# nicolapiccinelli/libmpc

Hardware: AMD Instinct MI355X
Metric: MPC solves/sec (whole node) + p50 solve latency, quadrotor LMPC N=20 batch=4096 (higher is better)
Workload: dtype f64; 1 GPU; quadrotor_ex.cpp LMPC nx=12 nu=4 ny=12 ph=ch=20, batch 4096 per GPU, SplitMix64 x0/u0/yref (SURVEY 8d), maximum_iteration=250; parallelism=single GPU, rccl_ranks=0, streams=1

## Files before the change

include/mpcx.h:

```cpp
#ifndef MPCX_H
#define MPCX_H

#include <stdint.h>

#ifdef __cplusplus
extern "C" {
#endif

#define MPCX_OK              0
#define MPCX_E_INVALID      -1
#define MPCX_E_UNSUPPORTED  -2
#define MPCX_E_DEVICE       -3
#define MPCX_E_NUMERIC      -4
#define MPCX_E_STATE        -5

#define MPCX_STATUS_SUCCESS        0
#define MPCX_STATUS_MAX_ITERATION  1
#define MPCX_STATUS_INFEASIBLE     2
#define MPCX_STATUS_ERROR          3
#define MPCX_STATUS_UNKNOWN        4

#define MPCX_SOLVER_SOLVED               1
#define MPCX_SOLVER_SOLVED_INACCURATE    2
#define MPCX_SOLVER_MAX_ITER_REACHED    -2
// ... 211 lines not shown

#define MPCX_COMM_ID_BYTES 128
typedef struct mpcx_comm *mpcx_comm_t;
int mpcx_comm_get_unique_id(void *id_out );
int mpcx_comm_create(int device, int rank, int world, const void *id, mpcx_comm_t *out);
int mpcx_comm_destroy(mpcx_comm_t c);
int mpcx_comm_rank(mpcx_comm_t c);
int mpcx_comm_world(mpcx_comm_t c);
int mpcx_allgather_u(mpcx_comm_t c, const double *u_local, int rows_per_rank, int nu, double *u_all, void *stream);

typedef struct mpcx_lmpc_hetero *mpcx_lmpc_hetero_t;
int mpcx_lmpc_hetero_create(const mpcx_lmpc_t *controllers, int count, int device, mpcx_lmpc_hetero_t *out);
int mpcx_lmpc_hetero_create_ex(const mpcx_lmpc_t *controllers, int count, int device, int condense_on_host, mpcx_lmpc_hetero_t *out);
int mpcx_lmpc_hetero_destroy(mpcx_lmpc_hetero_t f);
int mpcx_lmpc_hetero_get_info(mpcx_lmpc_hetero_t f, int *count, int *active_words, int *m_ref, double *bytes_per_model);
int mpcx_lmpc_hetero_solve_batch(mpcx_lmpc_hetero_t f, const mpcx_lmpc_batch *b, const int32_t *model_index, void *stream);
int mpcx_lmpc_hetero_time_solve_batch(mpcx_lmpc_hetero_t f, const mpcx_lmpc_batch *b, const int32_t *model_index, void *stream,
                                      int repeats, float *ms_mean);

int mpcx_lmpc_set_total_batch(mpcx_lmpc_t h, int total);

int mpcx_lmpc_debug_time_kernels(mpcx_lmpc_t h, const mpcx_lmpc_batch *b, void *stream, int repeats, float *ms3);
int mpcx_lmpc_debug_get(mpcx_lmpc_t h, const char *name, double *out, int cap);
int mpcx_lmpc_debug_setup_counts(mpcx_lmpc_t h, int *full, int *refs);
int mpcx_lmpc_debug_use_fused(mpcx_lmpc_t h, int mode);
int mpcx_lmpc_debug_force_generic(mpcx_lmpc_t h, int on);
int mpcx_lmpc_debug_set_rounds(mpcx_lmpc_t h, int rounds0, int check_every);
int mpcx_lmpc_debug_set_cycle_buffer(mpcx_lmpc_t h, void *dev_ptr);
int mpcx_lmpc_loop_debug_replay(mpcx_lmpc_loop_t l, void *stream);
int mpcx_lmpc_loop_debug_tick(mpcx_lmpc_loop_t l, int *tick);
int mpcx_nlmpc_debug_set_tolerances(mpcx_nlmpc_t h, double tol_step, double tol_con);
int mpcx_nlmpc_debug_last_form(void);
int mpcx_nlmpc_last_form(mpcx_nlmpc_t h);
int mpcx_nlmpc_debug_get_ws(mpcx_nlmpc_t h, int instance, double *out, int cap, int *layout, int nlayout);
int mpcx_nlmpc_debug_generated_source(const mpcx_nlmpc_source *src, char *out, int cap);
int mpcx_nlmpc_debug_compile_source(const mpcx_nlmpc_source *src);
int mpcx_lmpc_hetero_debug_get(mpcx_lmpc_hetero_t f, int k, const char *name, double *out, int cap);

const char *mpcx_version(void);

#ifdef __cplusplus
}
#endif
#endif
```

libmpc_amd/_capi.py:

```python
from __future__ import annotations

import ctypes as C
import os

_HERE = os.path.dirname(os.path.abspath(__file__))
LIB_PATH = os.environ.get("MPCX_LIBRARY", os.path.join(_HERE, "libmpcx.so"))

OK = 0
E_INVALID, E_UNSUPPORTED, E_DEVICE, E_NUMERIC, E_STATE = -1, -2, -3, -4, -5
STATUS_SUCCESS, STATUS_MAX_ITERATION, STATUS_INFEASIBLE, STATUS_ERROR, STATUS_UNKNOWN = range(5)
REF_SHARED, REF_PER_INSTANCE, REF_PER_STEP = 0, 1, 2
REF_PREVIEW = 3


class Dims(C.Structure):
    _fields_ = [(n, C.c_int) for n in ("nx", "nu", "ndu", "ny", "ph", "ch")]


class LParams(C.Structure):
    _fields_ = [("maximum_iteration", C.c_int), ("time_limit", C.c_double), ("enable_warm_start", C.c_int),
                ("alpha", C.c_double), ("rho", C.c_double), ("eps_rel", C.c_double), ("eps_abs", C.c_double),
                ("eps_prim_inf", C.c_double), ("eps_dual_inf", C.c_double),
                ("verbose", C.c_int), ("adaptive_rho", C.c_int), ("polish", C.c_int)]

# ... 36 lines not shown


EXPORTS = [
    "mpcx_lmpc_create", "mpcx_lmpc_destroy", "mpcx_lparams_default", "mpcx_last_error",
    "mpcx_lmpc_set_state_space_model", "mpcx_lmpc_set_disturbances",
    "mpcx_lmpc_set_objective_weights", "mpcx_lmpc_set_objective_weights_slice",
    "mpcx_lmpc_set_state_bounds", "mpcx_lmpc_set_state_bounds_slice",
    "mpcx_lmpc_set_input_bounds", "mpcx_lmpc_set_input_bounds_slice",
    "mpcx_lmpc_set_output_bounds", "mpcx_lmpc_set_output_bounds_slice",
    "mpcx_lmpc_set_scalar_constraint_slice", "mpcx_lmpc_set_scalar_constraint_index",
    "mpcx_lmpc_set_references", "mpcx_lmpc_set_references_slice",
    "mpcx_lmpc_set_exogenous_inputs", "mpcx_lmpc_set_exogenous_inputs_slice",
    "mpcx_lmpc_set_optimizer_parameters", "mpcx_lmpc_set_strict_infeasibility", "mpcx_lmpc_setup", "mpcx_lmpc_solve_batch",
    "mpcx_lmpc_time_solve_batch", "mpcx_lmpc_solve_host", "mpcx_lmpc_get_info", "mpcx_version",
    "mpcx_lmpc_graph_create", "mpcx_lmpc_graph_launch", "mpcx_lmpc_graph_destroy",
    "mpcx_lmpc_loop_create", "mpcx_lmpc_loop_run", "mpcx_lmpc_loop_destroy", "mpcx_lmpc_loop_desc_size",
    "mpcx_nlmpc_create", "mpcx_nlmpc_destroy", "mpcx_nlmpc_get_dims", "mpcx_nlmpc_evaluate_batch",
    "mpcx_nlparams_default", "mpcx_nlmpc_set_optimizer_parameters", "mpcx_nlmpc_solve_batch", "mpcx_nlmpc_time_solve_batch", "mpcx_discretize_batch",
    "mpcx_nlmpc_set_state_bounds_slice", "mpcx_nlmpc_set_input_bounds_slice", "mpcx_nlmpc_solve_host",
    "mpcx_nlmpc_create_custom", "mpcx_nlmpc_create_from_source", "mpcx_nlmpc_set_input_scale", "mpcx_nlmpc_set_state_scale",
    "mpcx_comm_get_unique_id", "mpcx_comm_create", "mpcx_comm_destroy", "mpcx_comm_rank", "mpcx_comm_world", "mpcx_allgather_u",
    "mpcx_lmpc_hetero_create", "mpcx_lmpc_hetero_destroy", "mpcx_lmpc_hetero_get_info", "mpcx_lmpc_hetero_solve_batch",
    "mpcx_lmpc_hetero_time_solve_batch", "mpcx_lmpc_hetero_create_ex", "mpcx_lmpc_hetero_debug_get",
    "mpcx_lmpc_set_total_batch", "mpcx_lmpc_debug_time_kernels", "mpcx_lmpc_debug_get", "mpcx_lmpc_debug_setup_counts", "mpcx_lmpc_debug_use_fused",
    "mpcx_lmpc_debug_force_generic", "mpcx_lmpc_debug_set_rounds", "mpcx_lmpc_debug_set_cycle_buffer",
    "mpcx_lmpc_loop_debug_replay", "mpcx_lmpc_loop_debug_tick",
    "mpcx_nlmpc_debug_set_tolerances", "mpcx_nlmpc_debug_last_form", "mpcx_nlmpc_last_form", "mpcx_nlmpc_debug_get_ws", "mpcx_nlmpc_debug_generated_source", "mpcx_nlmpc_debug_compile_source",
]


class NLParams(C.Structure):
    _fields_ = [("maximum_iteration", C.c_int), ("time_limit", C.c_double), ("enable_warm_start", C.c_int),
                ("relative_ftol", C.c_double), ("relative_xtol", C.c_double), ("absolute_ftol", C.c_double),
                ("absolute_xtol", C.c_double), ("hard_constraints", C.c_int)]


class NlmpcBatch(C.Structure):
    _fields_ = [("batch", C.c_int), ("x0", C.c_void_p), ("u0", C.c_void_p), ("z_warm", C.c_void_p), ("cmd", C.c_void_p),
                ("cost", C.c_void_p), ("status", C.c_void_p), ("solver_status", C.c_void_p), ("is_feasible", C.c_void_p),
                ("iterations", C.c_void_p), ("z", C.c_void_p), ("seq_state", C.c_void_p), ("seq_input", C.c_void_p),
                ("seq_output", C.c_void_p), ("warm_curvature", C.c_int), ("multipliers", C.c_void_p), ("params", C.c_void_p)]


class NlmpcDims(C.Structure):
    _fields_ = [(n, C.c_int) for n in ("nx", "nu", "ph", "ch", "nz", "neq", "nineq", "jeq_w", "neq_user", "ny", "nbnd", "n_params")]


# ... 65 lines not shown
```

libmpc_amd/csrc/lmpc_device.hpp:

```cpp
#pragma once

#include <atomic>
#include <cstdint>
#include <initializer_list>

namespace mpcx {

constexpr int kMaxActive = 28;
constexpr int kSld = kMaxActive + 1;
__host__ __device__ inline int ws_capacity(int nz) { return nz > kMaxActive ? nz : kMaxActive; }

struct LmpcDev {
    int nx, nu, ndu, ny, ph, ch, nf, nz, mg;
    int ldz, ldg, ldy;
    int m_ref, neq_ref, active_words;
    int has_dist, n_fixed;
    int max_iter, polish, check_every, polish_rounds0, polish_rounds;
    int cost_direct;
    int cond_status;
    int strict_infeasible;
    double alpha, sigma, eps_abs, eps_rel, eps_prim_inf;
    int adaptive_rho; double rho_user;
    int stage_len, arena_len, lds_per_wave;
    int fast_slice;
    int wsld;
    const double *A, *B, *C, *Bd, *Dd;
    const double *Wy, *Wu, *Wdu;
    const double *yref_s, *uref_s, *duref_s, *dmeas_s;
    const double *lo0x, *hi0x, *lo0u, *hi0u, *lo0y, *hi0y, *sX, *sU;
    double s0lo, s0hi;
    const double *H, *Kinv, *Gr, *Gc, *Y;
    const double *lw, *uw, *rho_b;
    const double *lg0, *ug0, *rho_g;
    const int *g_kind, *g_step, *g_comp, *g_refrow;
    const int *f_kind, *f_step, *f_comp; const double *f_lo, *f_hi;
    const int *boxrow_ptr, *boxrow_ref; const double *boxrow_lo, *boxrow_hi;
    const int *blk;
    int kin, nxp, nup, nyp, ione, nz16, mg16, ns, ns16, kq16, rowsA, ldy16;
    const double *MA0, *MA1, *Ym, *slo, *shi;
    const double *MA0p, *MA1p, *Ymp;
    const double *Hp;
    int rowsF, nsp, fused_ok, group_ok;
    const double *MF0, *MF1;
};

struct LmpcBatchDev {
    int batch;
    const double *x0, *u0;
    const double *yref; long yref_bs, yref_ks;
    const double *uref; long uref_bs, uref_ks;
    const double *duref; long duref_bs, duref_ks;
    const double *dmeas; long dmeas_bs, dmeas_ks;
    double *cmd, *cost;
    int32_t *status, *solver_status, *is_feasible, *iterations;
    uint32_t *active_lower, *active_upper;
    double *seq_state, *seq_output, *seq_input;
    int32_t *polish_rounds, *active_count;
    const uint32_t *warm_lower, *warm_upper;
    int warm_shift;
    int fq_cap;
    int fused;
    int *fq;
    int *pcounter;
    int n_models;
    const int32_t *model_index;
    long long *dbg_cycles;
// ... 59 lines not shown
```

libmpc_amd/csrc/lmpc_fast.hip:

```cpp
#include "lmpc_kernel_common.hpp"
#include <cstddef>
#include <cstdlib>
#include <utility>

namespace mpcx {

namespace {

#ifndef MPCX_FAST_PF_MAXCAP
#define MPCX_FAST_PF_MAXCAP 12
#endif
#ifndef MPCX_FAST_RB
#define MPCX_FAST_RB 4
#endif
#ifndef MPCX_FAST_PF
#define MPCX_FAST_PF 4
#endif
#ifndef MPCX_FAST_PF_ALL
#define MPCX_FAST_PF_ALL 6
#endif
#ifndef MPCX_FAST_NBUF
#define MPCX_FAST_NBUF 3
#endif
#ifndef MPCX_FAST_RB_DEEP
// ... 937 lines not shown
        const gdp src = gl(Bt.fused == 2 ? M.MF1 : M.MF0);
        for (int k = 2 * (int)threadIdx.x; k < nmf; k += 2 * (int)blockDim.x) {
            const d2 v = ld2(src + k);
            *reinterpret_cast<double2 *>(smem + k) = make_double2(v.x, v.y);
        }
    }
    double *lwuw = smem + nmf;
    fast_load_box<CPZ>(M, lwuw);
    double *rec = lwuw + 2 * 128 * CPZ + (size_t)wave * M.fast_slice;
    const int nwaves = gridDim.x * kPersistWaves, shard = blockIdx.x & 7;
    int b = blockIdx.x * kPersistWaves + wave;
    while (b < Bt.batch) {
        solve_fast<CPZ, CPG, 1>(M, Bt, b, lane, rec, lwuw, glw(wsbase) + (size_t)b * M.wsld, smem);
        int n = 0;
        if (lane == 0) n = atomicAdd(counter + shard, 1);
        n = __builtin_amdgcn_readfirstlane(n);
        b = nwaves + shard + 8 * n;
    }
}

template <size_t BYTES>
__device__ __forceinline__ void kernarg_touch()
{
    static_assert(BYTES <= 16 * 64 && BYTES > 15 * 64, "kernarg_touch covers sixteen lines, the sixteenth must exist");
    const auto ka = __builtin_amdgcn_kernarg_segment_ptr();
    int t0, t1, t2, t3, t4, t5, t6, t7, t8, t9, t10, t11, t12, t13, t14, t15;
    asm volatile("s_load_dword %0, %16, 0x0\n\ts_load_dword %1, %16, 0x40\n\ts_load_dword %2, %16, 0x80\n\ts_load_dword %3, %16, 0xc0\n\t"
                 "s_load_dword %4, %16, 0x100\n\ts_load_dword %5, %16, 0x140\n\ts_load_dword %6, %16, 0x180\n\ts_load_dword %7, %16, 0x1c0\n\t"
                 "s_load_dword %8, %16, 0x200\n\ts_load_dword %9, %16, 0x240\n\ts_load_dword %10, %16, 0x280\n\ts_load_dword %11, %16, 0x2c0\n\t"
                 "s_load_dword %12, %16, 0x300\n\ts_load_dword %13, %16, 0x340\n\ts_load_dword %14, %16, 0x380\n\ts_load_dword %15, %16, 0x3c0\n\t"
                 "s_waitcnt lgkmcnt(0)"
                 : "=&s"(t0), "=&s"(t1), "=&s"(t2), "=&s"(t3), "=&s"(t4), "=&s"(t5), "=&s"(t6), "=&s"(t7), "=&s"(t8), "=&s"(t9), "=&s"(t10), "=&s"(t11),
                   "=&s"(t12), "=&s"(t13), "=&s"(t14), "=&s"(t15)
                 : "s"(ka)
                 : "memory");
}
#ifndef MPCX_GROUP_BALANCE
#define MPCX_GROUP_BALANCE 1
#endif

template <int CPZ> constexpr int kGroupWavesOf = CPZ == 1 ? 16 : 8;
constexpr int kGroupG2 = 5;
constexpr int kGroupG1 = 2;
template <int CPZ, int CPG>
__global__ __launch_bounds__(kGroupWavesOf<CPZ> * 64) void lmpc_solve_group(const LmpcDev Mv, const LmpcBatchDev Btv, double *wsbasev, const int variantv)
{
    constexpr int kGroupWaves = kGroupWavesOf<CPZ>;
    extern __shared__ __attribute__((aligned(16))) double smem[];
#if defined(MPCX_GROUP_CUT) && MPCX_GROUP_CUT == 0
    { return; }
#endif
    kernarg_touch<sizeof(LmpcDev) + sizeof(LmpcBatchDev) + sizeof(double *) + sizeof(int)>();
    const group_args_p ka = (group_args_p)__builtin_amdgcn_kernarg_segment_ptr();
    const LmpcDev &M = (const LmpcDev &)ka->M;
    const LmpcBatchDev &Bt = (const LmpcBatchDev &)ka->Bt;
    double *const wsbase = ka->wsbase;
    const int variant = ka->variant;
    const int lane = threadIdx.x & 63, wave = threadIdx.x >> 6;
    const int j = lane & 15, kq = lane >> 4;
    const int nx = M.nx, nu = M.nu, ny = M.ny;
    const int kin4 = M.kin >> 2, nz4 = M.nz16 >> 2;
    const int ldz = M.ldz, ldg = M.ldg, ldy = M.ldy;
    constexpr int ZP = 128 * CPZ, GPD = 128 * CPG;
    double *lwuw = smem;
    double *slices = lwuw + 2 * ZP;
    double *Bv = slices + (size_t)kGroupWaves * M.fast_slice;
    double *Bf = Bv + (size_t)kin4 * 64;
    double *c0s = Bf + (size_t)nz4 * 64;
    unsigned *bad = reinterpret_cast<unsigned *>(c0s + kGroupWaves * 16);
    const int outld = 8 + ((nu + 1) & ~1);
    double *outs = c0s + kGroupWaves * 16 + 16;
    double *mine = slices + (size_t)wave * M.fast_slice;
    const gdp MAp = gl(variant ? M.MA1p : M.MA0p), Ymp = GP(Ymp);
    const int ntile1 = M.rowsA >> 4, tg = M.nz16 >> 4, ts = tg + (M.mg16 >> 4), tq = ts + (M.ns16 >> 4);
    const int ntile2 = M.ldy16 >> 4;
    const int G1 = (kin4 + 3) >> 2, G2 = (nz4 + 3) >> 2;
    auto ld4 = [](gdp p) -> v4d { return *reinterpret_cast<const v4d MPCX_GAS *>(p); };
    const bool jlive = j < kGroupWaves;
    double *sj = slices + (size_t)(jlive ? j : 0) * M.fast_slice;
    double *t0j = sj, *gt0j = sj + ZP, *lgj = gt0j + GPD, *ugj = lgj + GPD, *fj = ugj + GPD;

    const int b0 = blockIdx.x * kGroupWaves;
    const int bj = b0 + (jlive ? j : kGroupWaves - 1);
    const int bc = bj < Bt.batch ? bj : Bt.batch - 1;
    auto gstamp = [&](int k) { if (Bt.dbg_cycles && lane == 0 && b0 + wave < Bt.batch) Bt.dbg_cycles[(size_t)(b0 + wave) * 8 + k] = (long long)__builtin_readcyclecounter(); };
    gstamp(4);

    auto vin_at = [&](int kb) -> double {
        const int k = 4 * kb + kq;
        gdp src = gl(Bt.x0);
        bool ld = false;
        if (k < M.nxp) { ld = k < nx; src = gl(Bt.x0) + ((size_t)bc * nx + k); }
        else if (k < M.nxp + M.nup) { const int c = k - M.nxp; ld = c < nu; src = gl(Bt.u0) + ((size_t)bc * nu + c); }
        else if (k < M.ione) { const int c = k - M.nxp - M.nup; ld = variant && c < ny; src = gl(Bt.yref) + ((size_t)bc * Bt.yref_bs + c); }
        double v = k == M.ione ? 1.0 : 0.0;
        if (ld) v = *src;
        return v;
    };
    const double vin0 = wave < kin4 ? vin_at(wave) : 0.0;
    const int ebx = 2 * (int)threadIdx.x;
    const bool boxok = ebx < ldz;
    d2 bxl = {0.0, 0.0}, bxu = {0.0, 0.0};
    if (ebx < ZP) { bxl = ld2(GP(lw) + (boxok ? ebx : 0)); bxu = ld2(GP(uw) + (boxok ? ebx : 0)); }
    const int t1 = wave < ntile1 ? wave : ntile1 - 1;
    v4d a1[kGroupG1];
#pragma unroll
    for (int g = 0; g < kGroupG1; ++g) a1[g] = ld4(MAp + (((size_t)t1 * G1 + (g < G1 ? g : 0)) * 64 + lane) * 4);
    double eblo[4], ebhi[4];
    {
        const bool ing = t1 >= tg && t1 < ts, ins = t1 >= ts && t1 < tq;
        const gdp plo = ing ? GP(lg0) + 16 * (t1 - tg) : GP(slo) + 16 * (ins ? t1 - ts : 0);
        const gdp phi = ing ? GP(ug0) + 16 * (t1 - tg) : GP(shi) + 16 * (ins ? t1 - ts : 0);
        const int lim = ing ? ldg - 16 * (t1 - tg) : (ins ? M.ns - 16 * (t1 - ts) : 0);
#pragma unroll
        for (int r = 0; r < 4; ++r) {
            const int row = 4 * r + kq;
            eblo[r] = 0.0; ebhi[r] = 0.0;
            if (row < lim) { eblo[r] = plo[row]; ebhi[r] = phi[row]; }
        }
    }
    const int t2 = wave < ntile2 ? wave : ntile2 - 1;
    v4d a2[kGroupG2];
#pragma unroll
    for (int g = 0; g < kGroupG2; ++g) a2[g] = ld4(Ymp + (((size_t)t2 * G2 + (g < G2 ? g : 0)) * 64 + lane) * 4);
    d2 eql[CPG], equ[CPG];
#pragma unroll
    for (int c = 0; c < CPG; ++c) {
        const int r = 128 * c + 2 * lane;
        eql[c] = d2{0.0, 0.0}; equ[c] = d2{1.0, 1.0};
        if (wave == kGroupWaves - 1) { eql[c] = ld2(GP(lg0) + (r < ldg ? r : 0)); equ[c] = ld2(GP(ug0) + (r < ldg ? r : 0)); }
    }

    fast_init_pads<CPZ, CPG>(mine, ldz, ldg, lane);
    if (wave < kin4) Bv[wave * 64 + lane] = vin0;
    for (int kb = wave + kGroupWaves; kb < kin4; kb += kGroupWaves) Bv[kb * 64 + lane] = vin_at(kb);
    if (ebx < ZP) {
        const double INF = __builtin_huge_val();
        *reinterpret_cast<double2 *>(lwuw + ebx) = boxok ? make_double2(bxl.x, bxl.y) : make_double2(-INF, -INF);
        *reinterpret_cast<double2 *>(lwuw + ZP + ebx) = boxok ? make_double2(bxu.x, bxu.y) : make_double2(INF, INF);
    }
    if (threadIdx.x < 16) bad[threadIdx.x] = 0u;
    __syncthreads();
    gstamp(7);
#if defined(MPCX_GROUP_CUT) && MPCX_GROUP_CUT == 1
// ... 25 lines not shown
                    if (jlive && row < ldz) fj[row] = acc[r];
                }
            } else if (t < ts) {
#pragma unroll
                for (int r = 0; r < 4; ++r) {
                    const int row = 16 * (t - tg) + 4 * r + kq;
                    if (jlive && row < ldg) {
                        const double l0 = PRE ? eblo[r] : GP(lg0)[row], u0 = PRE ? ebhi[r] : GP(ug0)[row];
                        lgj[row] = l0 - acc[r]; ugj[row] = u0 - acc[r];
                    }
                }
            } else if (t < tq) {
#pragma unroll
                for (int r = 0; r < 4; ++r) {
                    const int row = 16 * (t - ts) + 4 * r + kq;
                    if (row < M.ns) badl |= violates(acc[r], PRE ? eblo[r] : GP(slo)[row], PRE ? ebhi[r] : GP(shi)[row], M.eps_abs, M.eps_rel);
                }
            } else {
#pragma unroll
                for (int r = 0; r < 4; ++r) {
                    const int kb2 = 4 * (t - tq) + r;
                    if (kb2 < kin4) c0p = fma(0.5 * Bv[kb2 * 64 + lane], acc[r], c0p);
                }
            }
        };
        int *eqb = reinterpret_cast<int *>(outs + kGroupWaves * outld);
        if (wave < ntile1) tile1.template operator()<true>(wave);
        for (int t = wave + kGroupWaves; t < ntile1; t += kGroupWaves) tile1.template operator()<false>(t);
        if (badl && jlive) atomicOr(&bad[j], 1u);
        c0p += __shfl_xor(c0p, 16, 64);
        c0p += __shfl_xor(c0p, 32, 64);
        if (kq == 0) c0s[wave * 16 + j] = c0p;
        __syncthreads();
        gstamp(5);
#if defined(MPCX_GROUP_CUT) && MPCX_GROUP_CUT == 2
        { return; }
#endif

        auto tile2 = [&]<bool PRE>(const int t) {
            v4d acc = {0.0, 0.0, 0.0, 0.0};
            for (int g0 = 0; g0 < G2; g0 += kGroupG2) {
                v4d a[kGroupG2];
#pragma unroll
                for (int g = 0; g < kGroupG2; ++g) a[g] = (PRE && g0 == 0) ? a2[g] : ld4(Ymp + (((size_t)t * G2 + (g0 + g < G2 ? g0 + g : g0)) * 64 + lane) * 4);
#pragma unroll
                for (int g = 0; g < kGroupG2; ++g)
#pragma unroll
                    for (int e = 0; e < 4; ++e) {
                        const int kb = 4 * (g0 + g) + e;
                        if (kb < nz4) acc = __builtin_amdgcn_mfma_f64_16x16x4f64(a[g][e], Bf[kb * 64 + lane], acc, 0, 0, 0);
                    }
            }
#pragma unroll
            for (int r = 0; r < 4; ++r) {
                const int row = 16 * t + 4 * r + kq;
                if (!jlive) continue;
                if (row < ldz) t0j[row] = acc[r];
                else if (row < ldy) gt0j[row - ldz] = acc[r];
            }
        };
        if (wave < ntile2) tile2.template operator()<true>(wave);
        for (int t = wave + kGroupWaves; t < ntile2; t += kGroupWaves) tile2.template operator()<false>(t);
        if (wave == kGroupWaves - 1) {
            int bits = 0;
#pragma unroll
            for (int c = 0; c < CPG; ++c) {
                const bool ok = 128 * c + 2 * lane < ldg;
                bits |= ((ok && eql[c].x == equ[c].x) ? 1 : 0) << (2 * c) | ((ok && eql[c].y == equ[c].y) ? 1 : 0) << (2 * c + 1);
            }
            eqb[lane] = bits;
        }
        if (threadIdx.x < kGroupWaves) {
            double *tl = slices + (size_t)threadIdx.x * M.fast_slice + 2 * ZP + 3 * GPD;
            double c0 = 0.0;
            for (int w = 0; w < kGroupWaves; ++w) c0 += c0s[w * 16 + threadIdx.x];
            tl[0] = c0;
            tl[1] = bad[threadIdx.x] ? 1.0 : 0.0;
        }
        __syncthreads();
        const int eqbits = eqb[lane];
        int inst = wave;
#if MPCX_GROUP_BALANCE
        if (b0 + kGroupWaves <= Bt.batch) {
            const double *t0m = mine, *gt0m = mine + ZP, *lgm = gt0m + GPD, *ugm = lgm + GPD;
            auto over = [](double v, double lo, double hi) { return fmax(fmax(lo - v, v - hi), 0.0); };
            double sv = 0.0;
#pragma unroll
            for (int c = 0; c < CPZ; ++c) {
                const int e = 128 * c + 2 * lane;
                const double2 l = *reinterpret_cast<const double2 *>(lwuw + e), u = *reinterpret_cast<const double2 *>(lwuw + ZP + e), t = *reinterpret_cast<const double2 *>(t0m + e);
                sv += over(t.x, l.x, u.x) + over(t.y, l.y, u.y);
            }
#pragma unroll
            for (int c = 0; c < CPG; ++c) {
                const int r = 128 * c + 2 * lane;
                const double2 l = *reinterpret_cast<const double2 *>(lgm + r), u = *reinterpret_cast<const double2 *>(ugm + r), t = *reinterpret_cast<const double2 *>(gt0m + r);
                sv += over(t.x, l.x, u.x) + over(t.y, l.y, u.y);
            }
            sv = wave_sum(sv);
            double *keys = reinterpret_cast<double *>(bad);
            if (lane == 0) keys[wave] = sv;
            __syncthreads();
            const int me = lane & (kGroupWaves - 1), part = lane >> 4;
            const double ki = keys[me];
            int rank = 0;
#pragma unroll
            for (int q = 0; q < kGroupWaves / 4; ++q) {
                const int jj = (kGroupWaves / 4) * part + q;
                const double kj = keys[jj];
                rank += (kj > ki || (kj == ki && jj < me)) ? 1 : 0;
            }
            rank += __shfl_xor(rank, 16, 64);
            rank += __shfl_xor(rank, 32, 64);
            const int q = rank >> 2, sd = (q & 1) ? 3 - (rank & 3) : (rank & 3);
            inst = (int)__builtin_ctzll(__ballot(lane < kGroupWaves && 4 * q + sd == wave));
        }
#endif
        double *const slice_i = slices + (size_t)inst * M.fast_slice;
        const int b = b0 + inst;
        gstamp(6);
#if defined(MPCX_GROUP_CUT) && MPCX_GROUP_CUT == 3
        { return; }
#endif
        if (b < Bt.batch) solve_fast<CPZ, CPG, 2>(M, Bt, b, lane, slice_i, lwuw, glw(wsbase) + (size_t)b * M.wsld, nullptr, outs + inst * outld, eqbits);
        __syncthreads();
        {
            const int t = threadIdx.x;
            if (t < kGroupWaves && b0 + t < Bt.batch) {
                const double *o = outs + t * outld;
                const int bb = b0 + t;
                if (o[7] == 2.0) {
                    if (Bt.cost) glw(Bt.cost)[bb] = o[0];
                    if (Bt.status) glw(Bt.status)[bb] = (int)o[1];
                    if (Bt.solver_status) glw(Bt.solver_status)[bb] = (int)o[2];
                    if (Bt.is_feasible) glw(Bt.is_feasible)[bb] = (int)o[3];
                    if (Bt.iterations) glw(Bt.iterations)[bb] = 0;
                    if (Bt.polish_rounds) glw(Bt.polish_rounds)[bb] = (int)o[5];
                    if (Bt.active_count) glw(Bt.active_count)[bb] = (int)o[6];
                }
            }
            for (int e = t; e < kGroupWaves * nu; e += blockDim.x) {
                const int ti = e / nu, jj = e - ti * nu;
// ... 60 lines not shown
    else if (b.n_models > 0) hipLaunchKernelGGL(k2h, dim3(blocks), dim3(kWavesPerBlock * 64), ldsf, stream, m_dev, b, ws);
    else hipLaunchKernelGGL(k2, dim3(blocks), dim3(kWavesPerBlock * 64), ldsf, stream, m_dev, b, ws);
    return hipGetLastError() == hipSuccess ? 0 : -3;
}

}

int lmpc_fast_slice(const LmpcDev &m)
{
    const int cp = lmpc_kernel_variant(m.ldz, m.ldg);
    if (cp < 1) return 0;
    const int fixed = cp == 1 ? fast_slice_fixed<1, 1>() : (cp == 2 ? fast_slice_fixed<2, 2>() : fast_slice_fixed<4, 4>());
    const int scratch = m.kin > 2 * m.nx ? m.kin : 2 * m.nx;
    int n = (fixed + scratch + 1) / 2 * 2;
    while (n % 16 != 2) n += 2;
    return n;
}

size_t lmpc_group_lds_bytes(const LmpcDev &m)
{
    const int cp = lmpc_kernel_variant(m.ldz, m.ldg);
    if (cp != 1 && cp != 2) return 0;
    const int nw = cp == 1 ? 16 : 8;
    return ((size_t)2 * 128 * cp + (size_t)nw * m.fast_slice + (size_t)(m.kin / 4 + m.nz16 / 4) * 64 + (size_t)nw * 16 + 16 + (size_t)nw * (8 + ((m.nu + 1) & ~1)) + 32) * sizeof(double);
}

int lmpc_launch_fast(const LmpcDev &m, const LmpcDev *m_dev, const LmpcBatchDev &b, double *ws, void *stream, LmpcForm form)
{
    hipStream_t s = reinterpret_cast<hipStream_t>(stream);
    switch (lmpc_kernel_variant(m.ldz, m.ldg)) {
    case 1: return launch_fast_variant<1, 1>(m, m_dev, b, ws, s, form);
#ifndef MPCX_FAST_ONLY_CP1
    case 2: return launch_fast_variant<2, 2>(m, m_dev, b, ws, s, form);
    case 4: return launch_fast_variant<4, 4>(m, m_dev, b, ws, s, form);
#endif
    default: return -2;
    }
}

}
```

libmpc_amd/csrc/mpcx_capi.cpp:

```cpp
#include <hip/hip_runtime.h>

#include <cstdio>
#include <cstring>
#include <memory>
#include <atomic>
#include <chrono>
#include <string>
#include <thread>
#include <type_traits>
#include <vector>

#include "../../include/mpcx.h"
#include "lmpc_device.hpp"
#include "lmpc_model.hpp"

namespace {

thread_local std::string g_err;

int fail(int code, const std::string &msg)
{
    g_err = msg;
    return code;
}
// ... 118 lines not shown
    D.nz16 = o.nz16; D.mg16 = o.mg16; D.ns = o.ns; D.ns16 = o.ns16; D.kq16 = o.kq16; D.rowsA = o.rowsA; D.ldy16 = o.ldy16;
    D.fast_slice = mpcx::lmpc_fast_slice(D);
    D.MA0 = U.up(o.MA[0], rc); D.MA1 = U.up(o.MA[1], rc); D.Ym = U.up(o.Ym, rc);
    {
        std::vector<double> pk;
        auto packed = [&](const std::vector<double> &v, int rows, int K) -> const std::vector<double> & {
            pk.clear();
            if (!v.empty()) { pk.resize(mpcx::lmpc_packed_len(rows, K)); mpcx::lmpc_pack_mfma_tiles(v.data(), rows, K, pk.data()); }
            return pk;
        };
        D.MA0p = U.up(packed(o.MA[0], o.rowsA, o.kin), rc); D.MA1p = U.up(packed(o.MA[1], o.rowsA, o.kin), rc); D.Ymp = U.up(packed(o.Ym, o.ldy16, o.nz16), rc);
        std::vector<double> hpad;
        if (D.cost_direct && !o.MA[0].empty() && !o.H.empty()) {
            hpad.assign((size_t)o.nz16 * o.nz16, 0.0);
            for (int c = 0; c < o.nz; ++c)
                for (int r = 0; r < o.nz; ++r) hpad[(size_t)c * o.nz16 + r] = o.H[(size_t)c * o.ldz + r];
        }
        D.Hp = hpad.empty() ? nullptr : U.up(packed(hpad, o.nz16, o.nz16), rc);
    }
    D.MF0 = U.up(o.MF[0], rc); D.MF1 = U.up(o.MF[1], rc); D.rowsF = o.rowsF; D.nsp = o.nsp;
    D.fused_ok = (h->use_fused != 0 && mpcx::lmpc_kernel_variant(o.ldz, o.ldg) == 1 && o.rowsF <= 384 && !D.cost_direct) ? 1 : 0;
    const size_t ldsg = mpcx::lmpc_group_lds_bytes(D);
    const int cpv = mpcx::lmpc_kernel_variant(o.ldz, o.ldg);
    D.group_ok = (h->use_fused != 0 && ldsg > 0 && ldsg <= mpcx::lmpc_lds_limit() && ((cpv == 1 && !D.cost_direct) || (cpv == 2 && h->use_fused == 2))) ? 1 : 0;
    D.slo = U.up(o.slo, rc); D.shi = U.up(o.shi, rc);
}

struct SlabUploader {
    static constexpr size_t kDevRegion = (size_t)1 << 44;
    std::vector<char> host;
    size_t dev_bytes = 0;
    bool big_on_device = false;
    template <typename T>
    const T *up(const std::vector<T> &v, int &)
    {
        const size_t at = (host.size() + 15) / 16 * 16;
        host.resize(at + (v.size() ? v.size() : 1) * sizeof(T), 0);
        if (v.size()) std::memcpy(host.data() + at, v.data(), v.size() * sizeof(T));
        return reinterpret_cast<const T *>(at + 1);
    }
    const double *reserve_big(size_t n)
    {
        const size_t at = (dev_bytes + 15) / 16 * 16;
        dev_bytes = at + (n ? n : 1) * sizeof(double);
        return reinterpret_cast<const double *>(kDevRegion + at + 1);
    }
    template <typename T>
// ... 1068 lines not shown

int mpcx_lmpc_debug_force_generic(mpcx_lmpc_t h, int on)
{
    CHECK_H(h);
    h->force_generic = on != 0;
    return MPCX_OK;
}

int mpcx_lmpc_debug_set_rounds(mpcx_lmpc_t h, int rounds0, int check_every)
{
    CHECK_H(h);
    h->dbg_rounds0 = rounds0; h->dbg_check_every = check_every;
    h->dirty = true;
    return MPCX_OK;
}

int mpcx_lmpc_debug_set_cycle_buffer(mpcx_lmpc_t h, void *dev_ptr)
{
    CHECK_H(h);
    h->dbg_cycles = static_cast<long long *>(dev_ptr);
    return MPCX_OK;
}

int mpcx_lmpc_debug_get(mpcx_lmpc_t h, const char *name, double *out, int cap)
{
    CHECK_H(h);
    int rc = mpcx_lmpc_setup(h);
    if (rc != MPCX_OK) return rc;
    const auto &o = h->cond;
    const std::vector<double> *v = nullptr;
    std::vector<double> tmp;
    std::string n(name ? name : "");
    if (n == "H") v = &o.H; else if (n == "Kinv") v = &o.Kinv; else if (n == "Gr") v = &o.Gr;
    else if (n == "Gc") v = &o.Gc; else if (n == "Y") v = &o.Y; else if (n == "lw") v = &o.lw;
    else if (n == "uw") v = &o.uw; else if (n == "rho_b") v = &o.rho_b; else if (n == "lg0") v = &o.lg0;
    else if (n == "ug0") v = &o.ug0; else if (n == "rho_g") v = &o.rho_g;
    else if (n == "dims") {
        tmp = {(double)o.nz, (double)o.mg, (double)o.ldz, (double)o.ldg, (double)o.ldy, (double)o.nf,
               (double)o.n_ref, (double)o.m_ref, (double)o.neq_ref, (double)o.fixed_rows.size(),
               (double)h->dev.lds_per_wave, (double)(o.h_regularised ? 1 : 0)};
        v = &tmp;
    } else if (n == "MA0") v = &o.MA[0]; else if (n == "MA1") v = &o.MA[1]; else if (n == "Ym") v = &o.Ym;
    else if (n == "MA0p" || n == "MA1p" || n == "Ymp") {
        const std::vector<double> &src = n == "Ymp" ? o.Ym : o.MA[n == "MA1p" ? 1 : 0];
        const int rows = n == "Ymp" ? o.ldy16 : o.rowsA, K = n == "Ymp" ? o.nz16 : o.kin;
        if (!src.empty()) { tmp.resize(mpcx::lmpc_packed_len(rows, K)); mpcx::lmpc_pack_mfma_tiles(src.data(), rows, K, tmp.data()); }
        v = &tmp;
    } else if (n == "flags") {
        tmp = {(double)h->dev.cost_direct, (double)h->dev.group_ok, (double)h->dev.fused_ok};
        v = &tmp;
    } else if (n == "dims_maps") {
        tmp = {(double)o.kin, (double)o.nxp, (double)o.nup, (double)o.nyp, (double)o.ione, (double)o.nz16, (double)o.mg16,
               (double)o.ns, (double)o.ns16, (double)o.kq16, (double)o.rowsA, (double)o.ldy16};
        v = &tmp;
    } else if (n == "g_refrow") { tmp.assign(o.g_refrow.begin(), o.g_refrow.end()); v = &tmp; }
    else if (n == "g_step") { tmp.assign(o.g_step.begin(), o.g_step.end()); v = &tmp; }
    else if (n == "g_kind") { tmp.assign(o.g_kind.begin(), o.g_kind.end()); v = &tmp; }
    else if (n == "g_comp") { tmp.assign(o.g_comp.begin(), o.g_comp.end()); v = &tmp; }
    else if (n == "fallback") {
        tmp.assign(3, 0.0);
        if (out && !h->host_only) {
            if (hipSetDevice(h->device) != hipSuccess || !fallback_state(h->scratch, tmp.data())) return fail(MPCX_E_DEVICE, "hipMemcpy failed");
        }
        v = &tmp;
    }
    else return fail(MPCX_E_INVALID, "unknown array name");
    if (!out) return (int)v->size();
    if (cap < (int)v->size()) return fail(MPCX_E_INVALID, "buffer too small");
    std::memcpy(out, v->data(), sizeof(double) * v->size());
    return (int)v->size();
}

}
// ... 1 lines not shown
```

Baseline: 126.4 million solves/s.

## Phase group-kernel tile work with host-built load-balanced schedule across waves

Splits the first matrix-tile phase so that only the tiles feeding the next stage run before the barrier. The remaining phase-1 tiles are interleaved with phase-2 tiles according to a greedy, SIMD-balanced schedule computed on the host and passed through kernel arguments. Balance keys are computed inside the tile-2 epilogue instead of a separate pass, and the cross-row reductions use permlane swaps instead of shuffles. The cost is a larger kernarg block (one more cache line to touch), extra LDS, per-tile reductions of the constant term, and a fallback path when the schedule does not fit.

```diff
diff --git a/include/mpcx.h b/include/mpcx.h
--- a/include/mpcx.h
+++ b/include/mpcx.h
@@ -257,6 +257,7 @@
 
 int mpcx_lmpc_debug_time_kernels(mpcx_lmpc_t h, const mpcx_lmpc_batch *b, void *stream, int repeats, float *ms3);
 int mpcx_lmpc_debug_get(mpcx_lmpc_t h, const char *name, double *out, int cap);
+int mpcx_lmpc_debug_group_schedule(int ts, int ntile1, int ntile2, int kin4, int nz4, int waves, unsigned char *out64);
 int mpcx_lmpc_debug_setup_counts(mpcx_lmpc_t h, int *full, int *refs);
 int mpcx_lmpc_debug_use_fused(mpcx_lmpc_t h, int mode);
 int mpcx_lmpc_debug_force_generic(mpcx_lmpc_t h, int on);
diff --git a/libmpc_amd/_capi.py b/libmpc_amd/_capi.py
--- a/libmpc_amd/_capi.py
+++ b/libmpc_amd/_capi.py
@@ -82,7 +82,7 @@
     "mpcx_comm_get_unique_id", "mpcx_comm_create", "mpcx_comm_destroy", "mpcx_comm_rank", "mpcx_comm_world", "mpcx_allgather_u",
     "mpcx_lmpc_hetero_create", "mpcx_lmpc_hetero_destroy", "mpcx_lmpc_hetero_get_info", "mpcx_lmpc_hetero_solve_batch",
     "mpcx_lmpc_hetero_time_solve_batch", "mpcx_lmpc_hetero_create_ex", "mpcx_lmpc_hetero_debug_get",
-    "mpcx_lmpc_set_total_batch", "mpcx_lmpc_debug_time_kernels", "mpcx_lmpc_debug_get", "mpcx_lmpc_debug_setup_counts", "mpcx_lmpc_debug_use_fused",
+    "mpcx_lmpc_set_total_batch", "mpcx_lmpc_debug_time_kernels", "mpcx_lmpc_debug_get", "mpcx_lmpc_debug_group_schedule", "mpcx_lmpc_debug_setup_counts", "mpcx_lmpc_debug_use_fused",
     "mpcx_lmpc_debug_force_generic", "mpcx_lmpc_debug_set_rounds", "mpcx_lmpc_debug_set_cycle_buffer",
     "mpcx_lmpc_loop_debug_replay", "mpcx_lmpc_loop_debug_tick",
     "mpcx_nlmpc_debug_set_tolerances", "mpcx_nlmpc_debug_last_form", "mpcx_nlmpc_last_form", "mpcx_nlmpc_debug_get_ws", "mpcx_nlmpc_debug_generated_source", "mpcx_nlmpc_debug_compile_source",
diff --git a/libmpc_amd/csrc/lmpc_device.hpp b/libmpc_amd/csrc/lmpc_device.hpp
--- a/libmpc_amd/csrc/lmpc_device.hpp
+++ b/libmpc_amd/csrc/lmpc_device.hpp
@@ -3,6 +3,8 @@
 #include <atomic>
 #include <cstdint>
 #include <initializer_list>
+
+#include "lmpc_group_schedule.hpp"
 
 namespace mpcx {
 
@@ -42,6 +44,7 @@
     const double *Hp;
     int rowsF, nsp, fused_ok, group_ok;
     const double *MF0, *MF1;
+    unsigned char gsched[kGroupSchedLen];
 };
 
 struct LmpcBatchDev {
diff --git a/libmpc_amd/csrc/lmpc_fast.hip b/libmpc_amd/csrc/lmpc_fast.hip
--- a/libmpc_amd/csrc/lmpc_fast.hip
+++ b/libmpc_amd/csrc/lmpc_fast.hip
@@ -983,22 +983,61 @@
 template <size_t BYTES>
 __device__ __forceinline__ void kernarg_touch()
 {
-    static_assert(BYTES <= 16 * 64 && BYTES > 15 * 64, "kernarg_touch covers sixteen lines, the sixteenth must exist");
+    static_assert(BYTES <= 17 * 64 && BYTES > 16 * 64, "kernarg_touch covers seventeen lines, the seventeenth must exist");
     const auto ka = __builtin_amdgcn_kernarg_segment_ptr();
-    int t0, t1, t2, t3, t4, t5, t6, t7, t8, t9, t10, t11, t12, t13, t14, t15;
-    asm volatile("s_load_dword %0, %16, 0x0\n\ts_load_dword %1, %16, 0x40\n\ts_load_dword %2, %16, 0x80\n\ts_load_dword %3, %16, 0xc0\n\t"
-                 "s_load_dword %4, %16, 0x100\n\ts_load_dword %5, %16, 0x140\n\ts_load_dword %6, %16, 0x180\n\ts_load_dword %7, %16, 0x1c0\n\t"
-                 "s_load_dword %8, %16, 0x200\n\ts_load_dword %9, %16, 0x240\n\ts_load_dword %10, %16, 0x280\n\ts_load_dword %11, %16, 0x2c0\n\t"
-                 "s_load_dword %12, %16, 0x300\n\ts_load_dword %13, %16, 0x340\n\ts_load_dword %14, %16, 0x380\n\ts_load_dword %15, %16, 0x3c0\n\t"
+    int t0, t1, t2, t3, t4, t5, t6, t7, t8, t9, t10, t11, t12, t13, t14, t15, t16;
+    asm volatile("s_load_dword %0, %17, 0x0\n\ts_load_dword %1, %17, 0x40\n\ts_load_dword %2, %17, 0x80\n\ts_load_dword %3, %17, 0xc0\n\t"
+                 "s_load_dword %4, %17, 0x100\n\ts_load_dword %5, %17, 0x140\n\ts_load_dword %6, %17, 0x180\n\ts_load_dword %7, %17, 0x1c0\n\t"
+                 "s_load_dword %8, %17, 0x200\n\ts_load_dword %9, %17, 0x240\n\ts_load_dword %10, %17, 0x280\n\ts_load_dword %11, %17, 0x2c0\n\t"
+                 "s_load_dword %12, %17, 0x300\n\ts_load_dword %13, %17, 0x340\n\ts_load_dword %14, %17, 0x380\n\ts_load_dword %15, %17, 0x3c0\n\t"
+                 "s_load_dword %16, %17, 0x400\n\t"
                  "s_waitcnt lgkmcnt(0)"
                  : "=&s"(t0), "=&s"(t1), "=&s"(t2), "=&s"(t3), "=&s"(t4), "=&s"(t5), "=&s"(t6), "=&s"(t7), "=&s"(t8), "=&s"(t9), "=&s"(t10), "=&s"(t11),
-                   "=&s"(t12), "=&s"(t13), "=&s"(t14), "=&s"(t15)
+                   "=&s"(t12), "=&s"(t13), "=&s"(t14), "=&s"(t15), "=&s"(t16)
                  : "s"(ka)
                  : "memory");
 }
 #ifndef MPCX_GROUP_BALANCE
 #define MPCX_GROUP_BALANCE 1
 #endif
+
+#ifndef MPCX_GROUP_PHASED
+#define MPCX_GROUP_PHASED 1
+#endif
+#ifndef MPCX_GROUP_EPIKEYS
+#define MPCX_GROUP_EPIKEYS 1
+#endif
+#ifndef MPCX_GROUP_SWAPSUM
+#define MPCX_GROUP_SWAPSUM 1
+#endif
+__device__ __forceinline__ double rows_sum(double v)
+{
+#if MPCX_GROUP_SWAPSUM
+    const unsigned lo = (unsigned)__double2loint(v), hi = (unsigned)__double2hiint(v);
+    const auto l16 = __builtin_amdgcn_permlane16_swap(lo, lo, false, false), h16 = __builtin_amdgcn_permlane16_swap(hi, hi, false, false);
+    v = __hiloint2double((int)h16[0], (int)l16[0]) + __hiloint2double((int)h16[1], (int)l16[1]);
+    const unsigned lo2 = (unsigned)__double2loint(v), hi2 = (unsigned)__double2hiint(v);
+    const auto l32 = __builtin_amdgcn_permlane32_swap(lo2, lo2, false, false), h32 = __builtin_amdgcn_permlane32_swap(hi2, hi2, false, false);
+    return __hiloint2double((int)h32[0], (int)l32[0]) + __hiloint2double((int)h32[1], (int)l32[1]);
+#else
+    v += __shfl_xor(v, 16, 64);
+    v += __shfl_xor(v, 32, 64);
+    return v;
+#endif
+}
+__device__ __forceinline__ int rows_sum(int v)
+{
+#if MPCX_GROUP_SWAPSUM
+    const auto a = __builtin_amdgcn_permlane16_swap((unsigned)v, (unsigned)v, false, false);
+    v = (int)(a[0] + a[1]);
+    const auto b = __builtin_amdgcn_permlane32_swap((unsigned)v, (unsigned)v, false, false);
+    return (int)(b[0] + b[1]);
+#else
+    v += __shfl_xor(v, 16, 64);
+    v += __shfl_xor(v, 32, 64);
+    return v;
+#endif
+}
 
 template <int CPZ> constexpr int kGroupWavesOf = CPZ == 1 ? 16 : 8;
 constexpr int kGroupG2 = 5;
@@ -1031,6 +1070,7 @@
     unsigned *bad = reinterpret_cast<unsigned *>(c0s + kGroupWaves * 16);
     const int outld = 8 + ((nu + 1) & ~1);
     double *outs = c0s + kGroupWaves * 16 + 16;
+    constexpr bool kPhased = MPCX_GROUP_PHASED != 0, kEpiKeys = MPCX_GROUP_EPIKEYS != 0;
     double *mine = slices + (size_t)wave * M.fast_slice;
     const gdp MAp = gl(variant ? M.MA1p : M.MA0p), Ymp = GP(Ymp);
     const int ntile1 = M.rowsA >> 4, tg = M.nz16 >> 4, ts = tg + (M.mg16 >> 4), tq = ts + (M.ns16 >> 4);
@@ -1041,7 +1081,9 @@
     double *sj = slices + (size_t)(jlive ? j : 0) * M.fast_slice;
     double *t0j = sj, *gt0j = sj + ZP, *lgj = gt0j + GPD, *ugj = lgj + GPD, *fj = ugj + GPD;
 
+    double *kpart = outs + kGroupWaves * outld + 32;
     const int b0 = blockIdx.x * kGroupWaves;
+    const bool dealt = b0 + kGroupWaves <= Bt.batch;
     const int bj = b0 + (jlive ? j : kGroupWaves - 1);
     const int bc = bj < Bt.batch ? bj : Bt.batch - 1;
     auto gstamp = [&](int k) { if (Bt.dbg_cycles && lane == 0 && b0 + wave < Bt.batch) Bt.dbg_cycles[(size_t)(b0 + wave) * 8 + k] = (long long)__builtin_readcyclecounter(); };
@@ -1063,7 +1105,11 @@
     const bool boxok = ebx < ldz;
     d2 bxl = {0.0, 0.0}, bxu = {0.0, 0.0};
     if (ebx < ZP) { bxl = ld2(GP(lw) + (boxok ? ebx : 0)); bxu = ld2(GP(uw) + (boxok ? ebx : 0)); }
-    const int t1 = wave < ntile1 ? wave : ntile1 - 1;
+    const int wv = __builtin_amdgcn_readfirstlane(wave);
+    const int code0 = kPhased ? (int)M.gsched[wv] : (int)kGroupSchedNone;
+    const bool b0p2 = code0 < kGroupSchedP1, b0p1 = !b0p2 && code0 != kGroupSchedNone;
+    const bool pre1b = kPhased && wave >= ts && b0p1;
+    const int t1 = kPhased ? (wave < ts ? wave : (pre1b ? (code0 & 0x7F) : ntile1 - 1)) : (wave < ntile1 ? wave : ntile1 - 1);
     v4d a1[kGroupG1];
 #pragma unroll
     for (int g = 0; g < kGroupG1; ++g) a1[g] = ld4(MAp + (((size_t)t1 * G1 + (g < G1 ? g : 0)) * 64 + lane) * 4);
@@ -1080,7 +1126,7 @@
             if (row < lim) { eblo[r] = plo[row]; ebhi[r] = phi[row]; }
         }
     }
-    const int t2 = wave < ntile2 ? wave : ntile2 - 1;
+    const int t2 = kPhased ? (b0p2 ? code0 : ntile2 - 1) : (wave < ntile2 ? wave : ntile2 - 1);
     v4d a2[kGroupG2];
 #pragma unroll
     for (int g = 0; g < kGroupG2; ++g) a2[g] = ld4(Ymp + (((size_t)t2 * G2 + (g < G2 ? g : 0)) * 64 + lane) * 4);
@@ -1152,15 +1198,30 @@
                     const int kb2 = 4 * (t - tq) + r;
                     if (kb2 < kin4) c0p = fma(0.5 * Bv[kb2 * 64 + lane], acc[r], c0p);
                 }
+                if constexpr (kPhased) {
+                    const double c0t = rows_sum(c0p);
+                    if (kq == 0) c0s[(t - tq) * 16 + j] = c0t;
+                    c0p = 0.0;
+                }
             }
         };
         int *eqb = reinterpret_cast<int *>(outs + kGroupWaves * outld);
-        if (wave < ntile1) tile1.template operator()<true>(wave);
-        for (int t = wave + kGroupWaves; t < ntile1; t += kGroupWaves) tile1.template operator()<false>(t);
-        if (badl && jlive) atomicOr(&bad[j], 1u);
-        c0p += __shfl_xor(c0p, 16, 64);
-        c0p += __shfl_xor(c0p, 32, 64);
-        if (kq == 0) c0s[wave * 16 + j] = c0p;
+        if constexpr (kPhased) {
+            if (wave < ts) {
+                tile1.template operator()<true>(wave);
+                for (int t = wave + kGroupWaves; t < ts; t += kGroupWaves) tile1.template operator()<false>(t);
+#pragma unroll
+                for (int g = 0; g < kGroupG1; ++g) asm volatile("" : "=v"(a1[g][0]), "=v"(a1[g][1]), "=v"(a1[g][2]), "=v"(a1[g][3]));
+#pragma unroll
+                for (int r = 0; r < 4; ++r) asm volatile("" : "=v"(eblo[r]), "=v"(ebhi[r]));
+            }
+        } else {
+            if (wave < ntile1) tile1.template operator()<true>(wave);
+            for (int t = wave + kGroupWaves; t < ntile1; t += kGroupWaves) tile1.template operator()<false>(t);
+            if (badl && jlive) atomicOr(&bad[j], 1u);
+            c0p = rows_sum(c0p);
+            if (kq == 0) c0s[wave * 16 + j] = c0p;
+        }
         __syncthreads();
         gstamp(5);
 #if defined(MPCX_GROUP_CUT) && MPCX_GROUP_CUT == 2
@@ -1188,9 +1249,38 @@
                 if (row < ldz) t0j[row] = acc[r];
                 else if (row < ldy) gt0j[row - ldz] = acc[r];
             }
+            if constexpr (kEpiKeys && MPCX_GROUP_BALANCE) {
+                if (dealt) {
+                    auto over = [](double v, double lo, double hi) { return fmax(fmax(lo - v, v - hi), 0.0); };
+                    double kp = 0.0;
+#pragma unroll
+                    for (int r = 0; r < 4; ++r) {
+                        const int row = 16 * t + 4 * r + kq;
+                        if (row < ldz) kp += over(acc[r], lwuw[row], lwuw[ZP + row]);
+                        else if (row < ldy) kp += over(acc[r], lgj[row - ldz], ugj[row - ldz]);
+                    }
+                    kp = rows_sum(kp);
+                    if (kq == 0) kpart[t * 16 + j] = kp;
+                }
+            }
         };
-        if (wave < ntile2) tile2.template operator()<true>(wave);
-        for (int t = wave + kGroupWaves; t < ntile2; t += kGroupWaves) tile2.template operator()<false>(t);
+        if constexpr (kPhased) {
+            if (code0 != kGroupSchedNone) {
+                if (b0p2) tile2.template operator()<true>(code0);
+                else if (pre1b) tile1.template operator()<true>(code0 & 0x7F);
+                else tile1.template operator()<false>(code0 & 0x7F);
+                for (int s = 1; s < kGroupSchedLen / kGroupWaves; ++s) {
+                    const int c = M.gsched[s * kGroupWaves + wv];
+                    if (c == kGroupSchedNone) break;
+                    if (c & kGroupSchedP1) tile1.template operator()<false>(c & 0x7F);
+                    else tile2.template operator()<false>(c);
+                }
+            }
+            if (badl && jlive) atomicOr(&bad[j], 1u);
+        } else {
+            if (wave < ntile2) tile2.template operator()<true>(wave);
+            for (int t = wave + kGroupWaves; t < ntile2; t += kGroupWaves) tile2.template operator()<false>(t);
+        }
         if (wave == kGroupWaves - 1) {
             int bits = 0;
 #pragma unroll
@@ -1200,7 +1290,7 @@
             }
             eqb[lane] = bits;
         }
-        if (threadIdx.x < kGroupWaves) {
+        if (!kPhased && threadIdx.x < kGroupWaves) {
             double *tl = slices + (size_t)threadIdx.x * M.fast_slice + 2 * ZP + 3 * GPD;
             double c0 = 0.0;
             for (int w = 0; w < kGroupWaves; ++w) c0 += c0s[w * 16 + threadIdx.x];
@@ -1211,7 +1301,25 @@
         const int eqbits = eqb[lane];
         int inst = wave;
 #if MPCX_GROUP_BALANCE
-        if (b0 + kGroupWaves <= Bt.batch) {
+        if (dealt) {
+            const int me = lane & (kGroupWaves - 1), part = lane >> 4;
+            int rank = 0;
+#if MPCX_GROUP_EPIKEYS
+            constexpr int KQ = kGroupWaves / 4;
+            double ki = 0.0, kj[KQ];
+#pragma unroll
+            for (int q = 0; q < KQ; ++q) kj[q] = 0.0;
+            for (int t = 0; t < ntile2; ++t) {
+                ki += kpart[t * 16 + me];
+#pragma unroll
+                for (int q = 0; q < KQ; ++q) kj[q] += kpart[t * 16 + KQ * part + q];
+            }
+#pragma unroll
+            for (int q = 0; q < KQ; ++q) {
+                const int jj = KQ * part + q;
+                rank += (kj[q] > ki || (kj[q] == ki && jj < me)) ? 1 : 0;
+            }
+#else
             const double *t0m = mine, *gt0m = mine + ZP, *lgm = gt0m + GPD, *ugm = lgm + GPD;
             auto over = [](double v, double lo, double hi) { return fmax(fmax(lo - v, v - hi), 0.0); };
             double sv = 0.0;
@@ -1228,26 +1336,30 @@
                 sv += over(t.x, l.x, u.x) + over(t.y, l.y, u.y);
             }
             sv = wave_sum(sv);
-            double *keys = reinterpret_cast<double *>(bad);
+            double *keys = kpart;
             if (lane == 0) keys[wave] = sv;
             __syncthreads();
-            const int me = lane & (kGroupWaves - 1), part = lane >> 4;
             const double ki = keys[me];
-            int rank = 0;
 #pragma unroll
             for (int q = 0; q < kGroupWaves / 4; ++q) {
                 const int jj = (kGroupWaves / 4) * part + q;
                 const double kj = keys[jj];
                 rank += (kj > ki || (kj == ki && jj < me)) ? 1 : 0;
             }
-            rank += __shfl_xor(rank, 16, 64);
-            rank += __shfl_xor(rank, 32, 64);
+#endif
+            rank = rows_sum(rank);
             const int q = rank >> 2, sd = (q & 1) ? 3 - (rank & 3) : (rank & 3);
             inst = (int)__builtin_ctzll(__ballot(lane < kGroupWaves && 4 * q + sd == wave));
         }
 #endif
         double *const slice_i = slices + (size_t)inst * M.fast_slice;
         const int b = b0 + inst;
+        if constexpr (kPhased) {
+            const int nq = ntile1 - tq, twrap = (ntile1 - 1) / kGroupWaves * kGroupWaves, nhi = twrap > tq ? ntile1 - twrap : 0;
+            double c0 = 0.0;
+            for (int i = 0; i < nq; ++i) c0 += c0s[((i < nhi ? twrap + i : tq + i - nhi) - tq) * 16 + inst];
+            if (lane == 0) *reinterpret_cast<double2 *>(slice_i + 2 * ZP + 3 * GPD) = make_double2(c0, bad[inst] ? 1.0 : 0.0);
+        }
         gstamp(6);
 #if defined(MPCX_GROUP_CUT) && MPCX_GROUP_CUT == 3
         { return; }
@@ -1354,7 +1466,7 @@
     const int cp = lmpc_kernel_variant(m.ldz, m.ldg);
     if (cp != 1 && cp != 2) return 0;
     const int nw = cp == 1 ? 16 : 8;
-    return ((size_t)2 * 128 * cp + (size_t)nw * m.fast_slice + (size_t)(m.kin / 4 + m.nz16 / 4) * 64 + (size_t)nw * 16 + 16 + (size_t)nw * (8 + ((m.nu + 1) & ~1)) + 32) * sizeof(double);
+    return ((size_t)2 * 128 * cp + (size_t)nw * m.fast_slice + (size_t)(m.kin / 4 + m.nz16 / 4) * 64 + (size_t)nw * 16 + 16 + (size_t)nw * (8 + ((m.nu + 1) & ~1)) + 32 + (size_t)(m.ldy16 / 16) * 16) * sizeof(double);
 }
 
 int lmpc_launch_fast(const LmpcDev &m, const LmpcDev *m_dev, const LmpcBatchDev &b, double *ws, void *stream, LmpcForm form)
diff --git a/libmpc_amd/csrc/lmpc_group_schedule.hpp b/libmpc_amd/csrc/lmpc_group_schedule.hpp
--- /dev/null
+++ b/libmpc_amd/csrc/lmpc_group_schedule.hpp
@@ -0,0 +1,41 @@
+#pragma once
+
+namespace mpcx {
+
+constexpr int kGroupSchedLen = 64;
+constexpr unsigned char kGroupSchedNone = 0xFF, kGroupSchedP1 = 0x80;
+
+inline int lmpc_group_schedule(const int ts, const int ntile1, const int ntile2, const int kin4, const int nz4, const int waves, unsigned char *out)
+{
+    for (int i = 0; i < kGroupSchedLen; ++i) out[i] = kGroupSchedNone;
+    if (waves < 4 || waves % 4 != 0 || kGroupSchedLen % waves != 0 || ts < 0 || ts > ntile1 || ntile2 < 0) return 0;
+    const int nrest = ntile1 - ts, slots = kGroupSchedLen / waves;
+    if (ntile2 + nrest > kGroupSchedLen || ntile2 > 0x7F || ntile1 > 0x7F) return 0;
+    int load[4] = {0, 0, 0, 0}, count[kGroupSchedLen] = {0};
+    bool greedy_fits = true;
+    const bool p2first = nz4 >= kin4;
+    for (int pass = 0; pass < 2 && greedy_fits; ++pass) {
+        const bool p2 = (pass == 0) == p2first;
+        const int n = p2 ? ntile2 : nrest, cost = p2 ? nz4 : kin4;
+        for (int i = 0; i < n; ++i) {
+            int sd = 0;
+            for (int s = 1; s < 4; ++s) if (load[s] < load[sd]) sd = s;
+            int w = sd;
+            for (int v = sd + 4; v < waves; v += 4) if (count[v] < count[w]) w = v;
+            if (count[w] >= slots) { greedy_fits = false; break; }
+            out[count[w] * waves + w] = (unsigned char)(p2 ? i : (kGroupSchedP1 | (ts + i)));
+            ++count[w]; load[sd] += cost;
+        }
+    }
+    if (greedy_fits) return 1;
+    for (int i = 0; i < kGroupSchedLen; ++i) out[i] = kGroupSchedNone;
+    int at = 0;
+    for (int pass = 0; pass < 2; ++pass) {
+        const bool p2 = (pass == 0) == p2first;
+        const int n = p2 ? ntile2 : nrest;
+        for (int i = 0; i < n; ++i, ++at) out[at] = (unsigned char)(p2 ? i : (kGroupSchedP1 | (ts + i)));
+    }
+    return 1;
+}
+
+}
diff --git a/libmpc_amd/csrc/mpcx_capi.cpp b/libmpc_amd/csrc/mpcx_capi.cpp
--- a/libmpc_amd/csrc/mpcx_capi.cpp
+++ b/libmpc_amd/csrc/mpcx_capi.cpp
@@ -164,7 +164,9 @@
     D.fused_ok = (h->use_fused != 0 && mpcx::lmpc_kernel_variant(o.ldz, o.ldg) == 1 && o.rowsF <= 384 && !D.cost_direct) ? 1 : 0;
     const size_t ldsg = mpcx::lmpc_group_lds_bytes(D);
     const int cpv = mpcx::lmpc_kernel_variant(o.ldz, o.ldg);
-    D.group_ok = (h->use_fused != 0 && ldsg > 0 && ldsg <= mpcx::lmpc_lds_limit() && ((cpv == 1 && !D.cost_direct) || (cpv == 2 && h->use_fused == 2))) ? 1 : 0;
+    const int gwaves = cpv == 1 ? 16 : 8;
+    const int gsched_ok = mpcx::lmpc_group_schedule((o.nz16 + o.mg16) / 16, o.rowsA / 16, o.ldy16 / 16, o.kin / 4, o.nz16 / 4, gwaves, D.gsched) && o.kq16 / 16 <= gwaves;
+    D.group_ok = (h->use_fused != 0 && ldsg > 0 && ldsg <= mpcx::lmpc_lds_limit() && gsched_ok && ((cpv == 1 && !D.cost_direct) || (cpv == 2 && h->use_fused == 2))) ? 1 : 0;
     D.slo = U.up(o.slo, rc); D.shi = U.up(o.shi, rc);
 }
 
@@ -1279,6 +1281,12 @@
     return MPCX_OK;
 }
 
+int mpcx_lmpc_debug_group_schedule(int ts, int ntile1, int ntile2, int kin4, int nz4, int waves, unsigned char *out64)
+{
+    if (!out64) return fail(MPCX_E_INVALID, "null output");
+    return mpcx::lmpc_group_schedule(ts, ntile1, ntile2, kin4, nz4, waves, out64);
+}
+
 int mpcx_lmpc_debug_get(mpcx_lmpc_t h, const char *name, double *out, int cap)
 {
     CHECK_H(h);
@@ -1306,6 +1314,13 @@
     } else if (n == "flags") {
         tmp = {(double)h->dev.cost_direct, (double)h->dev.group_ok, (double)h->dev.fused_ok};
         v = &tmp;
+    } else if (n == "group_schedule") {
+        const int cpv = mpcx::lmpc_kernel_variant(o.ldz, o.ldg), gwaves = cpv == 1 ? 16 : 8;
+        unsigned char tab[mpcx::kGroupSchedLen];
+        const int ok = mpcx::lmpc_group_schedule((o.nz16 + o.mg16) / 16, o.rowsA / 16, o.ldy16 / 16, o.kin / 4, o.nz16 / 4, gwaves, tab);
+        tmp = {(double)ok, (double)gwaves};
+        for (unsigned char c : tab) tmp.push_back((double)c);
+        v = &tmp;
     } else if (n == "dims_maps") {
         tmp = {(double)o.kin, (double)o.nxp, (double)o.nup, (double)o.nyp, (double)o.ione, (double)o.nz16, (double)o.mg16,
                (double)o.ns, (double)o.ns16, (double)o.kq16, (double)o.rowsA, (double)o.ldy16};
```

Result: slower. 124.3 million solves/s (-1.6%).
